# yakovdan/Background-Subtraction

Measured on NVIDIA B200. Metric: frames/s decomposed, higher is better.
Workload: dtype f32 (state) / exact int8-slice Gram on tcgen05 + f64 eigensolve

## Files before the change

background-subtraction_b200/csrc/gram_i8.cu:

```cuda
#include <cooperative_groups.h>
#include <stdio.h>
#include <math.h>
#include <algorithm>
#include <vector>
#include "common.cuh"
#include "kernels.h"
#include "tma.cuh"

namespace cg = cooperative_groups;

namespace bsub {

constexpr int GI_THREADS = 256;
constexpr int GI_KB = 64;
constexpr int GI_STAGES = 3;
constexpr int GI_FLUSH_KB = 448;
constexpr int GI_TILE_BYTES = 128 * GI_KB;
constexpr int GI_STAGE_BYTES = 8 * GI_TILE_BYTES;

struct GramI8Args {
    int n, nblk;
    const int4* cta_info;
    int nkb;
    const int* blk_n;
// ... 204 lines not shown
    asm volatile("{\n\t.reg .pred e;\n\telect.sync _|e, 0xffffffff;\n\t"
                 "@e tcgen05.commit.cta_group::1.mbarrier::arrive::one.shared::cluster.multicast::cluster.b64 [%0], %1;\n\t}"
                 ::"r"(smem_u32(bar)), "h"(cta_mask) : "memory");
}

__global__ void __launch_bounds__(GI_THREADS, 1)
gram_i8_c3_kernel(const __grid_constant__ CUtensorMap mapQ, GramI8C3Args a) {
    if (a.st != nullptr && (a.st->done || a.st->gram_mode != a.require_mode)) return;
    cg::cluster_group cluster = cg::this_cluster();
    extern __shared__ __align__(1024) unsigned char gi_smem[];
    unsigned char* stages = gi_smem;
    uint64_t* full = reinterpret_cast<uint64_t*>(gi_smem + (size_t)GI_STAGES * GI_STAGE_BYTES);
    uint64_t* empty = full + GI_STAGES;
    uint64_t* mine = empty + GI_STAGES;
    uint64_t* tmem_full = mine + GI_STAGES;
    uint64_t* tmem_empty = tmem_full + 1;
    uint32_t* tmem_base_s = reinterpret_cast<uint32_t*>(tmem_empty + 1);

    const int warp = __shfl_sync(0xffffffffu, (int)(threadIdx.x >> 5), 0), lane = threadIdx.x & 31;
    const int rank = (int)cluster.block_rank();
    const int cid = blockIdx.x / 3;
    const bool tX = cid < a.nX;
    const int kb0 = tX ? cid : cid - a.nX, kstride = tX ? a.nX : a.nY;
    const int nkb = (a.nkb > kb0) ? (a.nkb - kb0 + kstride - 1) / kstride : 0;
    const int bi = tX ? (rank == 2 ? 1 : 0) : rank;
    const int bj = tX ? (rank == 0 ? 1 : 2) : rank;
    const bool diag = !tX;
    int ld0_slot, ld0_blk, ld1_slot = -1, ld1_blk = 0; uint16_t ld0_mask, ld1_mask = 0;
    uint16_t sup_mask; int n_consumers;
    if (tX) {
        if (rank == 0)      { ld0_slot = 0; ld0_blk = 0; ld0_mask = 0x3; ld1_slot = 1; ld1_blk = 1; ld1_mask = 0x1; sup_mask = 0x1; n_consumers = 2; }
        else if (rank == 1) { ld0_slot = 1; ld0_blk = 2; ld0_mask = 0x6; sup_mask = 0x3; n_consumers = 2; }
        else                { ld0_slot = 0; ld0_blk = 1; ld0_mask = 0x4; sup_mask = 0x6; n_consumers = 1; }
    } else { ld0_slot = 0; ld0_blk = rank; ld0_mask = (uint16_t)(1u << rank); sup_mask = ld0_mask; n_consumers = 1; }

    if (threadIdx.x == 0) {
        for (int s = 0; s < GI_STAGES; ++s) { mbar_init(&full[s], 1); mbar_init(&empty[s], n_consumers); mbar_init(&mine[s], 1); }
        mbar_init(tmem_full, 1);
        mbar_init(tmem_empty, 128);
        mbar_fence_init();
        tma_prefetch_desc(&mapQ);
    }
    if (warp == 2) {
        asm volatile("tcgen05.alloc.cta_group::1.sync.aligned.shared::cta.b32 [%0], %1;" ::"r"(smem_u32(tmem_base_s)), "r"(512u) : "memory");
        asm volatile("tcgen05.relinquish_alloc_permit.cta_group::1.sync.aligned;" ::: "memory");
    }
    asm volatile("tcgen05.fence::before_thread_sync;" ::: "memory");
    cluster.sync();
    asm volatile("tcgen05.fence::after_thread_sync;" ::: "memory");
    const uint32_t tmem_base = __shfl_sync(0xffffffffu, *tmem_base_s, 0);

    if (warp == 0) {
        if (lane == 0) {
            const uint32_t tx = (uint32_t)(tX ? 8 : 4) * GI_TILE_BYTES;
            for (int kb = 0; kb < nkb; ++kb) {
                const int s = kb % GI_STAGES;
                const int u = kb / GI_STAGES;
                if (u > 0) gi_mbar_wait(&mine[s], (uint32_t)((u - 1) & 1));
                mbar_expect_tx(&full[s], tx);
                if (u > 0) gi_mbar_wait(&empty[s], (uint32_t)((u - 1) & 1));
                unsigned char* base = stages + (size_t)s * GI_STAGE_BYTES;
                const int k16 = (kb0 + kb * kstride) * (GI_KB / 16);
                for (int sl = 0; sl < 4; ++sl)
                    gi_tma_load_3d_mc(base + (size_t)(ld0_slot * 4 + sl) * GI_TILE_BYTES, &mapQ, &full[s], ld0_blk * 2 * a.nb, k16, sl, ld0_mask);
                if (ld1_slot >= 0)
                    for (int sl = 0; sl < 4; ++sl)
                        gi_tma_load_3d_mc(base + (size_t)(ld1_slot * 4 + sl) * GI_TILE_BYTES, &mapQ, &full[s], ld1_blk * 2 * a.nb, k16, sl, ld1_mask);
            }
        }
        __syncwarp();
    } else if (warp == 1) {
        {
            const uint32_t idesc = gi_instr_desc(a.N);
            const uint32_t offB = diag ? 0u : (uint32_t)(4 * GI_TILE_BYTES);
            const uint64_t desc0 = gi_smem_desc(0u, 2048u);
            int since_flush = 0, nflush = 0;
            for (int kb = 0; kb < nkb; ++kb) {
                const int s = kb % GI_STAGES;
                const int u = kb / GI_STAGES;
                if (since_flush == 0 && nflush > 0) {
                    gi_mbar_wait_w(tmem_empty, (uint32_t)((nflush - 1) & 1));
                    asm volatile("tcgen05.fence::after_thread_sync;" ::: "memory");
                }
                gi_mbar_wait_w(&full[s], (uint32_t)(u & 1));
                asm volatile("tcgen05.fence::after_thread_sync;" ::: "memory");
                const uint32_t sbase = smem_u32(stages + (size_t)s * GI_STAGE_BYTES);
                const uint64_t sa = desc0 + (uint64_t)((sbase >> 4) & 0x3FFF), sb = desc0 + (uint64_t)(((sbase + offB) >> 4) & 0x3FFF);
                if (!diag) {
#pragma unroll
                    for (int ks = 0; ks < GI_KB / 32; ++ks) {
#pragma unroll
                        for (int i = 0; i < 4; ++i)
#pragma unroll
                            for (int j = 0; j < 4; ++j) {
                                const int cls = i + j - 3;
                                if (cls < 0) continue;
                                const uint64_t da = sa + (uint64_t)((i * GI_TILE_BYTES + ks * 4096) >> 4);
                                const uint64_t db = sb + (uint64_t)((j * GI_TILE_BYTES + ks * 4096) >> 4);
                                const bool first = (since_flush == 0 && ks == 0 && j == 3);
                                gi_mma_w(tmem_base + (uint32_t)(cls * 128), da, db, idesc, first ? 0u : 1u);
                            }
                    }
                } else {
#pragma unroll
                    for (int ks = 0; ks < GI_KB / 32; ++ks) {
#pragma unroll
                        for (int i = 0; i < 4; ++i)
#pragma unroll
                            for (int j = 0; j < 4; ++j) {
                                const int cls = i + j - 3;
                                if (cls < 0) continue;
                                if (cls != 1 && i > j) continue;
                                const uint64_t da = sa + (uint64_t)((i * GI_TILE_BYTES + ks * 4096) >> 4);
                                const uint64_t db = sb + (uint64_t)((j * GI_TILE_BYTES + ks * 4096) >> 4);
                                const bool first = (since_flush == 0 && ks == 0 && j == 3);
                                gi_mma_w(tmem_base + (uint32_t)(cls * 128), da, db, idesc, first ? 0u : 1u);
                            }
                    }
                }
                gi_commit_mc_w(&empty[s], sup_mask);
                gi_commit_w(&mine[s]);
                ++since_flush;
                if (since_flush == GI_FLUSH_KB || kb == nkb - 1) {
                    gi_commit_w(tmem_full);
                    since_flush = 0; ++nflush;
                }
            }
        }
        __syncwarp();
    } else if (warp >= 4) {
        const int ew = warp - 4;
        const int nflush_total = (nkb + GI_FLUSH_KB - 1) / GI_FLUSH_KB;
        const int lrow = ew * 32 + lane;
        const int row = bi * a.nb + lrow;
        const bool row_ok = lrow < a.nb && row < a.n;
        const size_t ldg = (size_t)3 * 128;
        for (int fl = 0; fl < nflush_total; ++fl) {
            gi_mbar_wait(tmem_full, (uint32_t)(fl & 1));
            asm volatile("tcgen05.fence::after_thread_sync;" ::: "memory");
            for (int c0 = 0; c0 < a.N; c0 += 16) {
                uint32_t v3[16], v4[16], v5[16], v6[16];
                const uint32_t ta = tmem_base + ((uint32_t)(ew * 32) << 16) + (uint32_t)c0;
                gi_tmem_ld16(ta + 0 * 128, v3);
                gi_tmem_ld16(ta + 1 * 128, v4);
                gi_tmem_ld16(ta + 2 * 128, v5);
                gi_tmem_ld16(ta + 3 * 128, v6);
                asm volatile("tcgen05.wait::ld.sync.aligned;" ::: "memory");
                if (row_ok) {
#pragma unroll
                    for (int e = 0; e < 16; ++e) {
                        const int lcol = c0 + e, col = bj * a.nb + lcol;
                        if (lcol < a.nb && col < a.n) {
                            const long long half = (long long)(int)v3[e] + ((long long)(int)v5[e] << 16);
                            const long long whole = ((long long)(int)v4[e] << 8) + ((long long)(int)v6[e] << 24);
                            const long long val = half + whole;
                            if (val != 0) atomicAdd(a.Gint + (size_t)row * ldg + col, (unsigned long long)val);
                            if (diag && half != 0) atomicAdd(a.Gint + (size_t)col * ldg + row, (unsigned long long)half);
                        }
                    }
                }
            }
            asm volatile("tcgen05.fence::before_thread_sync;" ::: "memory");
            gi_mbar_arrive(tmem_empty);
        }
    }
    asm volatile("tcgen05.fence::before_thread_sync;" ::: "memory");
    cluster.sync();
    if (warp == 2) {
        asm volatile("tcgen05.dealloc.cta_group::1.sync.aligned.b32 %0, %1;" ::"r"(tmem_base), "r"(512u) : "memory");
    }
}

__global__ void __launch_bounds__(256) quantize_D_kernel(const float* __restrict__ D, long long ld, int n, long long ldq,
                                                         signed char* __restrict__ Wq, const double* __restrict__ dmax, DevState* st) {
    constexpr int QD_F = 32, QD_KB = 16;
    __shared__ uint4 stage[4][QD_KB][QD_F + 1];
    const double mx = *dmax;
    const double S = (mx > 0.0) ? exp2(ceil(log2(2.0 * mx))) : 1.0;
    if (blockIdx.x == 0 && threadIdx.x == 0) st->wq_scale = S;
    const float Qf = (float)(2147483648.0 / S);
    const long long nkb = ldq / 16, plane = ldq * (long long)n;
    const long long ntk = (nkb + QD_KB - 1) / QD_KB;
    const int ntf = (n + QD_F - 1) / QD_F;
    const long long ntiles = ntk * ntf;
    for (long long tile = blockIdx.x; tile < ntiles; tile += gridDim.x) {
        const long long kb0 = (tile / ntf) * QD_KB;
        const int f0 = (int)(tile % ntf) * QD_F;
#pragma unroll
        for (int pass = 0; pass < 8; ++pass) {
            const int idx = pass * 256 + threadIdx.x;
            const int fl = idx >> 6, q4 = idx & 63;
            const int f = f0 + fl;
            const long long p = kb0 * 16 + 4 * q4;
            float4 d = make_float4(0.f, 0.f, 0.f, 0.f);
            if (f < n && p < ld) d = ldg4_stream(D + (size_t)f * ld + p);
            const unsigned int u0 = ((unsigned int)__float2int_rn(d.x * Qf) + 0x00808080u) ^ 0x00808080u;
            const unsigned int u1 = ((unsigned int)__float2int_rn(d.y * Qf) + 0x00808080u) ^ 0x00808080u;
            const unsigned int u2 = ((unsigned int)__float2int_rn(d.z * Qf) + 0x00808080u) ^ 0x00808080u;
            const unsigned int u3 = ((unsigned int)__float2int_rn(d.w * Qf) + 0x00808080u) ^ 0x00808080u;
// ... 49 lines not shown
GramI8Plan make_gram_i8_plan(int n, long long ldq, int num_sms) {
    GramI8Plan p;
    p.n = n; p.ldq = ldq; p.m_real = 0; p.m_global = 0;
    p.nblk = (n + 127) / 128;
    p.nkb = (int)(ldq / GI_KB);
    p.smem_bytes = (size_t)GI_STAGES * GI_STAGE_BYTES + 256 + 1024;
    p.grid = num_sms;
    return p;
}

void fill_gram_i8_tables(const GramI8Plan& p, std::vector<int4>& cta_info, std::vector<int>& blk_n) {
    blk_n.assign(p.nblk, 128);
    const int last = p.n - (p.nblk - 1) * 128;
    blk_n[p.nblk - 1] = std::min(128, ((last + 15) / 16) * 16);
    std::vector<std::pair<int, int>> tiles;
    std::vector<double> w;
    double wsum = 0.0;
    for (int bi = 0; bi < p.nblk; ++bi)
        for (int bj = bi; bj < p.nblk; ++bj) {
            const double cost = 0.5 * (128.0 + (bi == bj ? 0.0 : (double)blk_n[bj])) / 256.0 +
                                0.5 * (bi == bj ? 0.7 : 1.0) * (double)blk_n[bj] / 128.0;
            tiles.push_back({bi, bj}); w.push_back(cost); wsum += cost;
        }
    std::vector<int> cnt(tiles.size(), 1);
    int left = p.grid - (int)tiles.size();
    if (left < 0) left = 0;
    std::vector<double> want(tiles.size());
    int given = 0;
    for (size_t t = 0; t < tiles.size(); ++t) { want[t] = w[t] / wsum * left; cnt[t] += (int)want[t]; given += (int)want[t]; }
    while (given < left) {
        size_t best = 0; double br = -1.0;
        for (size_t t = 0; t < tiles.size(); ++t) { double r = want[t] - (int)want[t]; if (r > br) { br = r; best = t; } }
        cnt[best]++; want[best] = (int)want[best]; ++given;
    }
    cta_info.clear();
    for (size_t t = 0; t < tiles.size(); ++t) {
        const int c = std::min(cnt[t], std::max(1, p.nkb));
        for (int k = 0; k < c; ++k) cta_info.push_back(make_int4(tiles[t].first, tiles[t].second, k, c));
    }
}

int gram_i8_last_block_n(const GramI8Plan& p) {
    const int last = p.n - (p.nblk - 1) * 128;
    return std::min(128, ((last + 15) / 16) * 16);
}

int make_gram_i8_map(const GramI8Plan& p, const signed char* Wq, CUtensorMap* map, int box_frames) {
    const uint64_t dims[3] = {(uint64_t)2 * p.n, (uint64_t)(p.ldq / 16), 4};
    const uint64_t strides[2] = {(uint64_t)16 * p.n, (uint64_t)p.ldq * (uint64_t)p.n};
    const uint32_t box[3] = {(uint32_t)(2 * box_frames), 4, 1};
    return make_tensor_map_u64(map, Wq, 3, dims, strides, box);
}

static int g_last_block_frames = 128;
int gram_i8_last_block_frames() { return g_last_block_frames; }

int launch_gram_i8(const GramI8Plan& p, const CUtensorMap& map, const CUtensorMap& map_last, const int4* cta_info_dev, int ncta, const int* blk_n_dev,
                   unsigned long long* Gint, double* G, int npad, const DevState* st, double scale_override, int require_mode,
                   cudaStream_t stream) {
    static unsigned long long attr_devs = 0;
    if (first_call_on_device(&attr_devs)) {
        BSUB_CUDA_CHECK(cudaFuncSetAttribute(gram_i8_kernel, cudaFuncAttributeMaxDynamicSharedMemorySize, (int)p.smem_bytes));
    }
    const double E_d = 5461.5 + 128.0 + 65536.0 * 5461.5 + 131072.0 * 0.25, E_o = 6.2e8;
    const double mg = (double)std::max(p.m_global, p.m_real);
    const double err_units = (p.m_real > 0) ? ((double)p.m_real / sqrt(mg)) * ((double)p.n + 3.0 * sqrt((double)p.n)) * E_o * 0x1p-24 : 0.0;
    const double diag_bias = (p.m_real > 0) ? (double)p.m_real * E_d * 0x1p-24 - err_units : 0.0;
    const size_t gbytes = sizeof(unsigned long long) * (size_t)p.nblk * 128 * p.nblk * 128;
    BSUB_CUDA_CHECK(cudaMemsetAsync(Gint, 0, gbytes, stream));
    static int c3_clusters = -1;
    if (p.nblk == 3 && c3_clusters != 0) {
        cudaLaunchConfig_t cfg = {};
        cudaLaunchAttribute at[1];
        at[0].id = cudaLaunchAttributeClusterDimension;
        at[0].val.clusterDim.x = 3; at[0].val.clusterDim.y = 1; at[0].val.clusterDim.z = 1;
        cfg.blockDim = dim3(GI_THREADS); cfg.dynamicSmemBytes = p.smem_bytes; cfg.stream = stream; cfg.attrs = at; cfg.numAttrs = 1;
        if (c3_clusters < 0) {
            c3_clusters = 0;
            if (getenv("BSUB_NO_GRAM_CLUSTER") == nullptr &&
                cudaFuncSetAttribute(gram_i8_c3_kernel, cudaFuncAttributeMaxDynamicSharedMemorySize, (int)p.smem_bytes) == cudaSuccess) {
                cfg.gridDim = dim3(3 * (p.grid / 3));
                int ncl = 0;
                if (cudaOccupancyMaxActiveClusters(&ncl, gram_i8_c3_kernel, &cfg) == cudaSuccess && ncl >= 2) c3_clusters = std::min(ncl, p.grid / 3);
            }
            (void)cudaGetLastError();
            if (getenv("BSUB_DEBUG")) fprintf(stderr, "gram_i8: %d multicast clusters of 3 CTAs\n", c3_clusters);
        }
        if (c3_clusters >= 2) {
            GramI8C3Args c;
            c.n = p.n; c.nkb = p.nkb;
            c.nb = (p.n + 2) / 3; c.N = ((c.nb + 15) / 16) * 16;
            c.nX = std::min(c3_clusters - 1, std::max(1, (int)lround(c3_clusters * 20.0 / 34.0))); c.nY = c3_clusters - c.nX;
            c.Gint = Gint; c.st = st; c.require_mode = require_mode;
            g_last_block_frames = c.nb;
            cfg.gridDim = dim3(3 * c3_clusters);
            BSUB_CUDA_CHECK(cudaLaunchKernelEx(&cfg, gram_i8_c3_kernel, map, c));
            gram_i8_finish_kernel<<<64, 256, 0, stream>>>(Gint, p.nblk, c.nb, p.n, npad, G, st, scale_override, require_mode, diag_bias, err_units,
                                                          (st != nullptr) ? G + (size_t)npad * npad + 8 : nullptr);
            BSUB_CUDA_CHECK(cudaGetLastError());
            return 0;
        }
    }
    GramI8Args a;
    a.n = p.n; a.nblk = p.nblk; a.nkb = p.nkb; a.cta_info = cta_info_dev; a.blk_n = blk_n_dev; a.Gint = Gint; a.st = st; a.require_mode = require_mode;
    gram_i8_kernel<<<ncta, GI_THREADS, p.smem_bytes, stream>>>(map, map_last, a);
    BSUB_CUDA_CHECK(cudaGetLastError());
    g_last_block_frames = 128;
    gram_i8_finish_kernel<<<64, 256, 0, stream>>>(Gint, p.nblk, 128, p.n, npad, G, st, scale_override, require_mode, diag_bias, err_units,
                                                          (st != nullptr) ? G + (size_t)npad * npad + 8 : nullptr);
    BSUB_CUDA_CHECK(cudaGetLastError());
    return 0;
}

}
```

background-subtraction_b200/csrc/kernels.h:

```cpp
#pragma once
#include <cuda.h>
#include <cuda_runtime.h>
#include <stddef.h>
#include <vector>
#include "common.cuh"

namespace bsub {

struct GramPlan {
    int n, npad, nb, ntasks, ntype, gridK, kc, nbox, boxrows;
    long long nchunks;
    size_t smem_bytes, partial_elems;
};
struct GramMaps { CUtensorMap D, S, Y; int narr; };
GramPlan make_gram_plan(int n, long long ld, int num_sms);
void fill_gram_tasks(const GramPlan& p, int2* host_tasks);
int make_gram_maps(const GramPlan& p, const float* D, const float* S, const float* Y, long long ld, GramMaps* maps);
int launch_gram(const GramPlan& p, const GramMaps& maps, bool combo, const int2* dev_tasks, const DevState* st,
                float inv_mu_override, double* partial, double* G, cudaStream_t stream);

struct GramI8Plan { int n, nblk, nkb, grid; long long ldq; size_t smem_bytes;
                    long long m_real;
                    long long m_global; };
GramI8Plan make_gram_i8_plan(int n, long long ldq, int num_sms);
void fill_gram_i8_tables(const GramI8Plan& p, std::vector<int4>& cta_info, std::vector<int>& blk_n);
int make_gram_i8_map(const GramI8Plan& p, const signed char* Wq, CUtensorMap* map, int box_frames);
int gram_i8_last_block_n(const GramI8Plan& p);
int gram_i8_last_block_frames();
int launch_quantize_D(const float* D, long long ld, int n, long long ldq, signed char* Wq, const double* dmax, DevState* st,
                      cudaStream_t stream);
int launch_gram_i8(const GramI8Plan& p, const CUtensorMap& map, const CUtensorMap& map_last, const int4* cta_info_dev, int ncta, const int* blk_n_dev,
                   unsigned long long* Gint, double* G, int npad, const DevState* st, double scale_override, int require_mode,
                   cudaStream_t stream);

struct EigPlan {
    int n, npad, C, rows_per, in_smem, kcap;
    size_t smem_bytes;
    size_t work_doubles;
};
struct EigBuffers {
    double* work;
    double* lam;
    double* Z;
    float* Vr;
    float* VC;
    int vstride;
};
EigPlan make_eig_plan(int n, int npad);
int launch_eig(const EigPlan& p, const double* G, const double* comm_max, EigBuffers b, DevState* st, int mode,
               int k_override, cudaStream_t stream);

struct ShrinkPlan {
    int n, rows, cols, R, P, Cf, nf, threads, grid_clusters, kr;
    long long ld, m;
    int ntile_r, ntile_c;
    long long ntiles;
    size_t smem_bytes;
    size_t tpart_floats;
    int nparts;
};
enum ShrinkMode { SHRINK_FLAT3 = 0, SHRINK_SPILL = 1, SHRINK_L1 = 2 };
ShrinkPlan make_shrink_plan(int n, int rows, int cols, long long ld, int num_sms, int R_hint, int Cf_hint);
struct ShrinkBuffers {
    const float* D; float* S; float* Y;
    float* T;
    float* U;
    float* tpart;
    const float* Vr; const float* VC; int vstride;
    double* part_zz;
    unsigned long long* part_nnz;
    float* part_max;
    float* part_wmax;
    int implied_first = 0;
    int have_flat = 0;
    const float* Tt = nullptr;
};
int launch_shrink(const ShrinkPlan& p, ShrinkBuffers b, const DevState* st, int mode, cudaStream_t stream);

struct ShrinkTmaPlan {
    int n, rows, cols, R, P, Cf, nf, KR, grid_clusters, nparts, ntile_r, ntile_c, bufstride, NT, occ;
    long long ld, ntiles;
    size_t smem_bytes, tpart_floats;
};
struct ShrinkTmaMaps { CUtensorMap D, S, Y, U, Q, Vr, VC; bool has_U, has_Q; };
bool make_shrink_tma_plan(int n, int rows, int cols, long long ld, int num_sms, int R_hint, int Cf_hint, ShrinkTmaPlan* out);
// ... 98 lines not shown
```

background-subtraction_b200/csrc/solver.cu:

```cuda
#include <math.h>
#include <stdarg.h>
#include <stdlib.h>
#include <string.h>
#include <vector>
#include <algorithm>
#include "../../include/bsub_b200.h"
#include "common.cuh"
#include "kernels.h"

namespace bsub {
static thread_local char g_err[1024] = "";
void set_error(const char* fmt, ...) {
    va_list ap;
    va_start(ap, fmt);
    vsnprintf(g_err, sizeof(g_err), fmt, ap);
    va_end(ap);
}
}

using namespace bsub;

#define CK(expr) BSUB_CUDA_CHECK(expr)
#define RET_IF(expr) do { int _rc = (expr); if (_rc != 0) return _rc; } while (0)

static const int kCommTail = 16;
static const int kRunAhead = 3;

struct bsub_solver {
    bsub_config cfg;
    int device = 0, num_sms = 148;
    long long m = 0, ld = 0;
    int n = 0, npad = 0;
    float *D = nullptr, *S = nullptr, *Y = nullptr, *T = nullptr, *L = nullptr, *U = nullptr;
    DevState* st = nullptr;
    IterLog* log = nullptr;
    HostMirror* mirror = nullptr;
    HostMirror* mirror_dev = nullptr;
    double* comm_sum = nullptr;
    double* comm_max = nullptr;
    GramPlan gp; GramMaps gmaps; int2* tasks_dev = nullptr; double* gram_partial = nullptr;
    EigPlan ep; EigBuffers eb;
    ShrinkPlan sp; ShrinkTmaPlan stp; ShrinkTmaMaps stmaps; bool use_tma = false, stmaps_ready = false;
    ShrinkStreamPlan ssp; ShrinkTmaMaps ssmaps; bool use_stream = false;
    bool use_i8 = false; signed char* Wq = nullptr; unsigned long long* Gint = nullptr; GramI8Plan gip; CUtensorMap gimap, gimap_last;
    int4* gi_info = nullptr; int* gi_blkn = nullptr; int gi_ncta = 0; float* part_wmax = nullptr;
    bool use_proj = false; ProjectPlan pjp; float* Tt = nullptr;
    bool use_flat = false, sfmaps_ready = false; ShrinkFlatPlan sfp; ShrinkFlatMaps sfmaps;
    bool force_S = false;
    int proj_iter = -1;
    float* tpart = nullptr; double* part_zz = nullptr; unsigned long long* part_nnz = nullptr;
    float* part_max = nullptr;
    int shrink_mode = SHRINK_FLAT3;
    int* gptr = nullptr; int* gidx = nullptr; int ngroups = 0; bool groups_set = false;
    float* eta_dev = nullptr; float* xi = nullptr; long long xi_floats = 0; float* tot = nullptr;
    float* xi2 = nullptr; float* tot2 = nullptr; int* sweeps2 = nullptr; long long xi2_floats = 0, tot2_floats = 0;
    int* sweeps_dev = nullptr; bool graph_set = false;
    int* pg_ints = nullptr; float* pg_eta = nullptr; GenericGraphDev pg_dev; GenericGraphLayout pg_layout; bool pg_bg = false;
    unsigned char* labels_dev = nullptr; double* lam_table = nullptr; double* bsums = nullptr; int nlab = 0; bool blocks_set = false;
    unsigned char* mask_stage = nullptr;
    double* mask_scratch = nullptr;
    double* stage64 = nullptr; size_t stage64_doubles = 0;
    cudaStream_t last_stream = nullptr; bool stream_seen = false;
    bool implied_first = false;
    bool loaded = false, finalized = false, initialised = false;
    cudaEvent_t ev[kRunAhead + 1];
    int iters_enqueued = 0;
};

static cudaStream_t as_stream(void* s) { return reinterpret_cast<cudaStream_t>(s); }
static cudaStream_t use_stream(bsub_solver* s, void* stream) {
    s->last_stream = as_stream(stream); s->stream_seen = true;
    return s->last_stream;
}
static int ensure_stage64(bsub_solver* s, size_t doubles) {
    if (s->stage64_doubles >= doubles) return 0;
    if (s->stage64) { cudaFree(s->stage64); s->stage64 = nullptr; s->stage64_doubles = 0; }
    BSUB_CUDA_CHECK(cudaMalloc((void**)&s->stage64, sizeof(double) * doubles));
    s->stage64_doubles = doubles;
    return 0;
}
struct DevScope {
    std::vector<void*> ptrs;
    ~DevScope() { for (void* p : ptrs) if (p) cudaFree(p); }
    template <typename T> int alloc(T** out, size_t bytes) {
        void* p = nullptr;
        if (cudaMalloc(&p, bytes ? bytes : 1) != cudaSuccess) { set_error("cudaMalloc(%zu) failed: %s", bytes, cudaGetErrorString(cudaGetLastError())); return -1; }
        ptrs.push_back(p);
        *out = reinterpret_cast<T*>(p);
        return 0;
    }
};

static int round_half_even_005(int d) {
    return (int)nearbyint(0.05 * (double)d);
}

extern "C" {
// ... 82 lines not shown
        if (make_gram_maps(s->gp, s->D, s->S, s->Y, s->ld, &s->gmaps) != 0) { rc = -1; break; }
        std::vector<int2> tasks(s->gp.ntasks);
        fill_gram_tasks(s->gp, tasks.data());
        ALLOC(s->tasks_dev, sizeof(int2) * s->gp.ntasks);
        cudaMemcpy(s->tasks_dev, tasks.data(), sizeof(int2) * s->gp.ntasks, cudaMemcpyHostToDevice);
        ALLOC(s->gram_partial, sizeof(double) * s->gp.partial_elems);
        s->ep = make_eig_plan(s->n, s->npad);
        ALLOC(s->eb.work, sizeof(double) * s->ep.work_doubles);
        ALLOC(s->eb.lam, sizeof(double) * s->n);
        ALLOC(s->eb.Z, sizeof(double) * (size_t)s->n * s->n);
        s->eb.vstride = std::max(16, ((s->n + 3) / 4) * 4);
        ALLOC(s->eb.Vr, sizeof(float) * (size_t)s->n * s->eb.vstride);
        ALLOC(s->eb.VC, sizeof(float) * (size_t)s->n * s->eb.vstride);
        cudaMemset(s->eb.Vr, 0, sizeof(float) * (size_t)s->n * s->eb.vstride);
        cudaMemset(s->eb.VC, 0, sizeof(float) * (size_t)s->n * s->eb.vstride);
        int rows = cfg->rows, cols = cfg->cols;
        if ((long long)rows * cols != s->m) {
            rows = (int)s->m; cols = 1;
            for (int r = 4096; r >= 48; r -= 4)
                if (s->m % r == 0) { rows = r; cols = (int)(s->m / r); break; }
        }
        s->sp = make_shrink_plan(s->n, rows, cols, s->ld, s->num_sms, cfg->tile_rows, cfg->cluster_frames);
        s->use_tma = (getenv("BSUB_NO_TMA") == nullptr) &&
                     make_shrink_tma_plan(s->n, rows, cols, s->ld, s->num_sms, cfg->tile_rows, cfg->cluster_frames, &s->stp);
        s->use_stream = s->use_tma && (getenv("BSUB_NO_STREAM") == nullptr) &&
                        make_shrink_stream_plan(s->n, rows, cols, s->ld, s->num_sms, cfg->tile_rows, &s->ssp);
        ALLOC(s->tpart, sizeof(float) * std::max(s->sp.tpart_floats, s->use_tma ? s->stp.tpart_floats : (size_t)0));
        int nparts = std::max(std::max(s->sp.nparts, (s->use_tma ? s->stp.nparts : 0) + (s->use_stream ? s->ssp.nparts : 0) + s->num_sms), s->num_sms * 8);
        ALLOC(s->part_zz, sizeof(double) * nparts); ALLOC(s->part_nnz, sizeof(unsigned long long) * nparts);
        ALLOC(s->part_max, sizeof(float) * nparts);
        cudaMemset(s->part_zz, 0, sizeof(double) * nparts); cudaMemset(s->part_nnz, 0, sizeof(unsigned long long) * nparts);
        cudaMemset(s->part_max, 0, sizeof(float) * nparts);
        s->use_i8 = s->use_stream && (shrink_stream_ldq(s->ssp) > 0) && (getenv("BSUB_NO_I8") == nullptr) &&
                    (cfg->prox == BSUB_PROX_FLAT_LINF || cfg->prox == BSUB_PROX_L1);
        if (s->use_i8) {
            const long long ldq = shrink_stream_ldq(s->ssp);
            s->gip = make_gram_i8_plan(s->n, ldq, s->num_sms);
            s->gip.m_real = (getenv("BSUB_NO_GRAM_BIAS") == nullptr) ? s->m : 0;
            s->gip.m_global = s->cfg.m_global;
            std::vector<int4> info; std::vector<int> blkn;
            fill_gram_i8_tables(s->gip, info, blkn);
            s->gi_ncta = (int)info.size();
            ALLOC(s->Wq, (size_t)4 * s->n * ldq);
            cudaMemset(s->Wq, 0, (size_t)4 * s->n * ldq);
            ALLOC(s->Gint, sizeof(unsigned long long) * (size_t)s->gip.nblk * 128 * s->gip.nblk * 128);
            ALLOC(s->gi_info, sizeof(int4) * info.size());
            ALLOC(s->gi_blkn, sizeof(int) * blkn.size());
            ALLOC(s->part_wmax, sizeof(float) * (s->ssp.grid + s->num_sms));
            cudaMemcpy(s->gi_info, info.data(), sizeof(int4) * info.size(), cudaMemcpyHostToDevice);
            cudaMemcpy(s->gi_blkn, blkn.data(), sizeof(int) * blkn.size(), cudaMemcpyHostToDevice);
            cudaMemset(s->part_wmax, 0, sizeof(float) * (s->ssp.grid + s->num_sms));
            if (make_gram_i8_map(s->gip, s->Wq, &s->gimap, 128) != 0) { rc = -1; break; }
            if (make_gram_i8_map(s->gip, s->Wq, &s->gimap_last, gram_i8_last_block_n(s->gip)) != 0) { rc = -1; break; }
            s->use_proj = (getenv("BSUB_NO_PROJ") == nullptr) && make_project_plan(s->n, s->ssp.R, ldq, s->num_sms, &s->pjp);
            if (s->use_proj) {
                const size_t tt = sizeof(float) * (size_t)s->ssp.ntiles * 16 * 4 * s->ssp.R;
                ALLOC(s->Tt, tt);
                cudaMemset(s->Tt, 0, tt);
                s->use_flat = (getenv("BSUB_NO_FLAT") == nullptr) && make_shrink_flat_plan(s->n, s->ssp.rows, s->ssp.cols, s->ld, s->num_sms, s->ssp, &s->sfp);
            }
        }
        for (int i = 0; i <= kRunAhead; ++i)
            if (cudaEventCreateWithFlags(&s->ev[i], cudaEventDisableTiming) != cudaSuccess) { set_error("bsub_create: event"); rc = -1; break; }
        if (rc) break;
        switch (cfg->prox) {
            case BSUB_PROX_FLAT_LINF: s->shrink_mode = (cfg->group_rows == 3 && cfg->group_cols == 3) ? SHRINK_FLAT3 : SHRINK_SPILL; break;
            case BSUB_PROX_L1: s->shrink_mode = SHRINK_L1; break;
            default: s->shrink_mode = SHRINK_SPILL; break;
        }
        s->implied_first = s->use_i8 && s->use_stream && s->shrink_mode != SHRINK_SPILL && s->cfg.use_sv_prediction &&
                           s->cfg.sv0 >= 1 && s->cfg.sv0 <= s->ssp.kcap && getenv("BSUB_NO_IMPLIED_FIRST") == nullptr;
        if (s->shrink_mode == SHRINK_SPILL) { ALLOC(s->U, mat); ALLOC(s->L, mat); cudaMemset(s->U, 0, mat); cudaMemset(s->L, 0, mat); }
#undef ALLOC
        if (cudaGetLastError() != cudaSuccess) {  }
    } while (0);
    if (rc != 0) { bsub_destroy(s); return rc; }
    *out = s;
    return 0;
}

int bsub_set_flat_groups(bsub_solver* s, const int32_t* g) {
    if (!s || !g) { set_error("bsub_set_flat_groups: null argument"); return -1; }
    if (s->cfg.prox != BSUB_PROX_FLAT_LINF) { set_error("bsub_set_flat_groups: solver was not created with BSUB_PROX_FLAT_LINF"); return -1; }
    const long long m = s->m;
    const int rows = s->cfg.rows, cols = s->cfg.cols;
    bool regular = ((long long)rows * cols == m);
    if (regular) {
        const int ntr = (rows + 2) / 3;
        for (int j = 0; j < cols && regular; ++j)
            for (int i = 0; i < rows; ++i)
                if (g[(long long)j * rows + i] != (j / 3) * ntr + (i / 3) + 1) { regular = false; break; }
    }
    s->groups_set = true;
    if (regular) { s->shrink_mode = SHRINK_FLAT3; return 0; }
    int gmax = 0;
    for (long long p = 0; p < m; ++p) { if (g[p] < 0) { set_error("bsub_set_flat_groups: negative group id"); return -1; } gmax = std::max(gmax, (int)g[p]); }
    std::vector<int> ptr((size_t)gmax + 1, 0), idx;
    for (long long p = 0; p < m; ++p) if (g[p] > 0) ptr[g[p]]++;
    std::vector<int> start((size_t)gmax + 1, 0);
    int acc = 0;
    for (int k = 1; k <= gmax; ++k) { start[k - 1] = acc; acc += ptr[k]; }
    start[gmax] = acc;
    idx.resize((size_t)std::max(acc, 1));
    std::vector<int> fill(start.begin(), start.end());
    for (long long p = 0; p < m; ++p) if (g[p] > 0) idx[fill[g[p] - 1]++] = (int)p;
    if (s->gptr) cudaFree(s->gptr);
// ... 184 lines not shown
    memset(&h, 0, sizeof(h));
    const bsub_config& c = s->cfg;
    const double mx = (double)std::max<long long>(c.m_global, c.n);
    h.lambda = 1.0 / (sqrt(mx) * c.delta);
    h.non_block_lambda = c.non_block_lambda_scale * h.lambda;
    h.rho = c.rho; h.tol = c.tol; h.mu_scale = c.mu_scale;
    h.max_iter = c.max_iter;
    h.d = c.d_global > 0 ? c.d_global : (int)std::min<long long>(c.m_global, c.n);
    h.round005d = round_half_even_005(h.d);
    h.use_sv_prediction = c.use_sv_prediction;
    h.break_on_rank0 = c.break_on_rank0;
    h.sv = c.use_sv_prediction ? c.sv0 : h.d;
    h.use_i8 = s->use_i8 ? 1 : 0;
    CK(cudaMemcpyAsync(s->st, &h, sizeof(h), cudaMemcpyHostToDevice, st));
    CK(cudaStreamSynchronize(st));
    memset((void*)s->mirror, 0, sizeof(HostMirror));
    return 0;
}

int bsub_set_always_store_S(bsub_solver* s, int on) {
    if (!s) { set_error("bsub_set_always_store_S: null solver"); return -1; }
    s->force_S = on != 0;
    return 0;
}

int bsub_comm_buffers(bsub_solver* s, double** sum_buf, int64_t* sum_count, double** max_buf, int64_t* max_count) {
    if (!s) { set_error("bsub_comm_buffers: null solver"); return -1; }
    if (sum_buf) *sum_buf = s->comm_sum;
    if (sum_count) *sum_count = (int64_t)s->npad * s->npad + kCommTail;
    if (max_buf) *max_buf = s->comm_max;
    if (max_count) *max_count = 8;
    return 0;
}

static int check_ready(bsub_solver* s) {
    if (!s) { set_error("null solver"); return -1; }
    if (!s->loaded) { set_error("no data loaded (call bsub_load_* first)"); return -1; }
    if (s->cfg.prox == BSUB_PROX_FLAT_LINF && !s->groups_set) { set_error("one of graphs or groups must not be None"); return -1; }
    if ((s->cfg.prox == BSUB_PROX_GRAPH_LINF || s->cfg.prox == BSUB_PROX_GRAPH_CENTER_BG || s->cfg.prox == BSUB_PROX_GRAPH_GENERIC) &&
        !s->graph_set) { set_error("one of graphs or groups must not be None"); return -1; }
    if (s->cfg.prox == BSUB_PROX_BLOCK_L2 && !s->blocks_set) { set_error("blocks_by_frame / lambdas_by_frame not set"); return -1; }
    return 0;
}

int bsub_step_init_local(bsub_solver* s, void* stream) {
    RET_IF(check_ready(s));
    cudaStream_t st = use_stream(s, stream);
    RET_IF(upload_state(s, st));
    CK(cudaMemsetAsync(s->comm_max, 0, sizeof(double) * 8, st));
    CK(cudaMemsetAsync(s->comm_sum + (size_t)s->npad * s->npad, 0, sizeof(double) * kCommTail, st));
    RET_IF(launch_rowsum_max(s->D, s->ld, s->m, s->n, s->comm_max, st));
    if (s->use_i8) {
        RET_IF(launch_quantize_D(s->D, s->ld, s->n, s->gip.ldq, s->Wq, s->comm_max + 2, s->st, st));
        RET_IF(launch_gram_i8(s->gip, s->gimap, s->gimap_last, s->gi_info, s->gi_ncta, s->gi_blkn, s->Gint, s->comm_sum, s->npad, s->st, 0.0, 0,
                              st));
    } else {
        RET_IF(launch_gram(s->gp, s->gmaps, false, s->tasks_dev, nullptr, 0.f, s->gram_partial, s->comm_sum, st));
    }
    s->iters_enqueued = 0;
    s->proj_iter = -1;
    s->finalized = false;
    return 0;
}

int bsub_step_init_finish(bsub_solver* s, void* stream) {
    RET_IF(check_ready(s));
    cudaStream_t st = use_stream(s, stream);
    RET_IF(launch_eig(s->ep, s->comm_sum, s->comm_max, s->eb, s->st, 0, 1, st));
    if (!s->implied_first) RET_IF(launch_init_Y(s->D, s->Y, s->S, s->ld, s->n, s->st, st));
    s->initialised = true;
    return 0;
}

int bsub_step_gram(bsub_solver* s, void* stream) {
    if (!s || !s->initialised) { set_error("bsub_step_gram: solver not initialised"); return -1; }
    use_stream(s, stream);
    RET_IF(launch_gram(s->gp, s->gmaps, true, s->tasks_dev, s->st, 0.f, s->gram_partial, s->comm_sum, as_stream(stream)));
    if (s->use_i8)
        RET_IF(launch_gram_i8(s->gip, s->gimap, s->gimap_last, s->gi_info, s->gi_ncta, s->gi_blkn, s->Gint, s->comm_sum, s->npad, s->st, 0.0, 1,
                              as_stream(stream)));
    return 0;
}

int bsub_step_solve(bsub_solver* s, void* stream) {
    if (!s || !s->initialised) { set_error("bsub_step_solve: solver not initialised"); return -1; }
    return launch_eig(s->ep, s->comm_sum, s->comm_max, s->eb, s->st, 1, 0, as_stream(stream));
}

int bsub_step_project(bsub_solver* s, void* stream) {
    if (!s || !s->initialised) { set_error("bsub_step_project: solver not initialised"); return -1; }
    cudaStream_t st = use_stream(s, stream);
    const bool proj = s->use_proj && s->use_stream && s->use_i8 && s->shrink_mode != SHRINK_SPILL;
    if (!proj || s->proj_iter == s->iters_enqueued) return 0;
    RET_IF(launch_project(s->pjp, s->Wq, s->eb.Vr, s->eb.vstride, s->T, s->ld, s->Tt, s->ssp.rows, s->ssp.cols, s->ssp.R, s->ssp.ntile_r,
                          s->ssp.ntiles, s->ssp.kcap, s->st, st));
    s->proj_iter = s->iters_enqueued;
    return 0;
}

static int step_shrink_impl(bsub_solver* s, void* stream, int part) {
    if (!s || !s->initialised) { set_error("bsub_step_shrink: solver not initialised"); return -1; }
    cudaStream_t st = use_stream(s, stream);
    const bool split = s->shrink_mode == SHRINK_SPILL && (s->cfg.prox == BSUB_PROX_BLOCK_L2 || s->cfg.prox == BSUB_PROX_GRAPH_LINF);
    if (part == 2 && !split) return 0;
    if (part == 2) {
        if (s->cfg.prox == BSUB_PROX_BLOCK_L2)
            RET_IF(launch_block_l2_apply(s->U, s->S, s->labels_dev, s->ld, s->m, s->n, s->nlab, s->bsums, s->lam_table, s->st, 0.0, 0.0, st));
        const int np2 = s->num_sms * 8;
        RET_IF(launch_dual_update(s->D, s->S, s->S, s->Y, s->T, s->eb.VC, s->eb.vstride, s->st, s->L, s->ld, s->n, s->part_zz,
                                  s->part_nnz, s->part_max, np2, st));
        RET_IF(launch_control_post(s->st, s->part_zz, s->part_nnz, s->part_max, np2, s->comm_sum + (size_t)s->npad * s->npad, s->log,
                                   s->mirror_dev, 1 | 4, nullptr, 0, st));
        return 0;
    }
    ShrinkBuffers b;
    b.D = s->D; b.S = s->S; b.Y = s->Y; b.T = s->T; b.U = s->U; b.tpart = s->tpart; b.Vr = s->eb.Vr; b.VC = s->eb.VC;
    b.vstride = s->eb.vstride; b.part_zz = s->part_zz; b.part_nnz = s->part_nnz; b.part_max = s->part_max;
    b.part_wmax = s->use_i8 ? s->part_wmax : nullptr;
    b.implied_first = s->implied_first ? 1 : 0;
    const bool proj = s->use_proj && s->use_stream && s->use_i8 && s->shrink_mode != SHRINK_SPILL;
    const bool flat = proj && s->use_flat;
    b.Tt = proj ? s->Tt : nullptr;
    b.have_flat = flat ? 1 : 0;
    int nparts = s->sp.nparts;
    if (s->use_tma) {
        if (!s->stmaps_ready) {
            RET_IF(make_shrink_tma_maps(s->stp, s->D, s->S, s->Y, s->U, &s->stmaps));
            if (s->use_stream) RET_IF(make_shrink_stream_maps(s->ssp, s->D, s->S, s->Y, s->U, &s->ssmaps));
            if (s->use_stream) RET_IF(make_shrink_stream_vmaps(s->ssp, s->eb.Vr, s->eb.VC, s->eb.vstride, &s->ssmaps));
            if (s->use_stream && s->use_i8) RET_IF(make_shrink_stream_qmap(s->ssp, s->Wq, &s->ssmaps));
            s->stmaps_ready = true;
        }
// ... 457 lines not shown

int bsub_gram_dev(const float* D, const float* S, const float* Y, int64_t ld, int64_t m, int32_t n, double mu, double* G_host,
                  void* stream) {
    if (!D || !G_host || ld < m || (ld % 32) != 0) { set_error("bsub_gram_dev: bad argument (ld must be a multiple of 32, pad columns zero)"); return -1; }
    if ((S == nullptr) != (Y == nullptr)) { set_error("bsub_gram_dev: S and Y must both be given or both be NULL"); return -1; }
    cudaStream_t st = as_stream(stream);
    int dev = 0, sms = 148;
    CK(cudaGetDevice(&dev));
    cudaDeviceGetAttribute(&sms, cudaDevAttrMultiProcessorCount, dev);
    GramPlan gp = make_gram_plan(n, ld, sms);
    std::vector<int2> tasks(gp.ntasks);
    fill_gram_tasks(gp, tasks.data());
    DevScope mem;
    int2* tasks_d = nullptr; double *partial = nullptr, *G = nullptr;
    RET_IF(mem.alloc(&tasks_d, sizeof(int2) * gp.ntasks));
    RET_IF(mem.alloc(&partial, sizeof(double) * gp.partial_elems));
    RET_IF(mem.alloc(&G, sizeof(double) * (size_t)gp.npad * gp.npad));
    CK(cudaMemcpy(tasks_d, tasks.data(), sizeof(int2) * gp.ntasks, cudaMemcpyHostToDevice));
    GramMaps gm;
    RET_IF(make_gram_maps(gp, D, S, Y, ld, &gm));
    RET_IF(launch_gram(gp, gm, S != nullptr, tasks_d, nullptr, (float)(S ? 1.0 / mu : 0.0), partial, G, st));
    CK(cudaMemcpy2DAsync(G_host, sizeof(double) * n, G, sizeof(double) * gp.npad, sizeof(double) * n, n, cudaMemcpyDeviceToHost, st));
    CK(cudaStreamSynchronize(st));
    return 0;
}

int bsub_gram_i8_test(const int8_t* slices_host, int32_t n, int64_t ldq, int64_t* G_host) {
    if (!slices_host || !G_host || n <= 0 || ldq <= 0 || (ldq % 64) != 0) { set_error("bsub_gram_i8_test: bad argument"); return -1; }
    int dev = 0, sms = 148;
    CK(cudaGetDevice(&dev));
    cudaDeviceGetAttribute(&sms, cudaDevAttrMultiProcessorCount, dev);
    GramI8Plan gp = make_gram_i8_plan(n, ldq, sms);
    std::vector<int4> info; std::vector<int> blkn;
    fill_gram_i8_tables(gp, info, blkn);
    DevScope mem;
    signed char* q = nullptr; int4* info_d = nullptr; int* blkn_d = nullptr; unsigned long long* Gint = nullptr; double* G = nullptr;
    const size_t qbytes = (size_t)4 * n * ldq, gn = (size_t)gp.nblk * 128;
    const int npad = ((n + 31) / 32) * 32;
    RET_IF(mem.alloc(&q, qbytes));
    RET_IF(mem.alloc(&info_d, sizeof(int4) * info.size()));
    RET_IF(mem.alloc(&blkn_d, sizeof(int) * blkn.size()));
    RET_IF(mem.alloc(&Gint, sizeof(unsigned long long) * gn * gn));
    RET_IF(mem.alloc(&G, sizeof(double) * (size_t)npad * npad));
    {
        std::vector<signed char> packed(qbytes);
        for (int sl = 0; sl < 4; ++sl)
            for (int f = 0; f < n; ++f)
                for (long long k = 0; k < ldq / 16; ++k)
                    memcpy(&packed[(((size_t)sl * (ldq / 16) + k) * n + f) * 16], &slices_host[((size_t)sl * n + f) * ldq + k * 16], 16);
        CK(cudaMemcpy(q, packed.data(), qbytes, cudaMemcpyHostToDevice));
    }
    CK(cudaMemcpy(info_d, info.data(), sizeof(int4) * info.size(), cudaMemcpyHostToDevice));
    CK(cudaMemcpy(blkn_d, blkn.data(), sizeof(int) * blkn.size(), cudaMemcpyHostToDevice));
    CUtensorMap map, map_last;
    RET_IF(make_gram_i8_map(gp, q, &map, 128));
    RET_IF(make_gram_i8_map(gp, q, &map_last, gram_i8_last_block_n(gp)));
    RET_IF(launch_gram_i8(gp, map, map_last, info_d, (int)info.size(), blkn_d, Gint, G, npad, nullptr, 1.0, 1, 0));
    CK(cudaDeviceSynchronize());
    std::vector<long long> tmp(gn * gn);
    CK(cudaMemcpy(tmp.data(), Gint, sizeof(long long) * gn * gn, cudaMemcpyDeviceToHost));
    for (int i = 0; i < n; ++i)
        for (int j = 0; j < n; ++j) {
            const int blk = gram_i8_last_block_frames();
            const int r = (i / blk <= j / blk) ? i : j, c = (i / blk <= j / blk) ? j : i;
            G_host[(size_t)i * n + j] = tmp[(size_t)r * gn + c];
        }
    return 0;
}

int bsub_gram_i8_bench(int32_t n, int64_t ldq, int32_t reps, float* ms_out) {
    if (!ms_out || n <= 0 || ldq <= 0 || (ldq % 64) != 0 || reps <= 0) { set_error("bsub_gram_i8_bench: bad argument"); return -1; }
    int dev = 0, sms = 148;
    CK(cudaGetDevice(&dev));
    cudaDeviceGetAttribute(&sms, cudaDevAttrMultiProcessorCount, dev);
    GramI8Plan gp = make_gram_i8_plan(n, ldq, sms);
    std::vector<int4> info; std::vector<int> blkn;
    fill_gram_i8_tables(gp, info, blkn);
    DevScope mem;
    signed char* q = nullptr; int4* info_d = nullptr; int* blkn_d = nullptr; unsigned long long* Gint = nullptr; double* G = nullptr;
    const size_t qbytes = (size_t)4 * n * ldq, gn = (size_t)gp.nblk * 128;
    const int npad = ((n + 31) / 32) * 32;
    RET_IF(mem.alloc(&q, qbytes));
    RET_IF(mem.alloc(&info_d, sizeof(int4) * info.size()));
    RET_IF(mem.alloc(&blkn_d, sizeof(int) * blkn.size()));
    RET_IF(mem.alloc(&Gint, sizeof(unsigned long long) * gn * gn));
    RET_IF(mem.alloc(&G, sizeof(double) * ((size_t)npad * npad + 16)));
    CK(cudaMemset(q, 0x35, qbytes));
    CK(cudaMemcpy(info_d, info.data(), sizeof(int4) * info.size(), cudaMemcpyHostToDevice));
    CK(cudaMemcpy(blkn_d, blkn.data(), sizeof(int) * blkn.size(), cudaMemcpyHostToDevice));
    CUtensorMap map, map_last;
    RET_IF(make_gram_i8_map(gp, q, &map, 128));
    RET_IF(make_gram_i8_map(gp, q, &map_last, gram_i8_last_block_n(gp)));
    cudaEvent_t e0, e1;
    CK(cudaEventCreate(&e0)); CK(cudaEventCreate(&e1));
    for (int r = 0; r < 2; ++r) RET_IF(launch_gram_i8(gp, map, map_last, info_d, (int)info.size(), blkn_d, Gint, G, npad, nullptr, 1.0, 1, 0));
    CK(cudaEventRecord(e0, 0));
    for (int r = 0; r < reps; ++r) RET_IF(launch_gram_i8(gp, map, map_last, info_d, (int)info.size(), blkn_d, Gint, G, npad, nullptr, 1.0, 1, 0));
    CK(cudaEventRecord(e1, 0));
    CK(cudaEventSynchronize(e1));
    float ms = 0.f;
    CK(cudaEventElapsedTime(&ms, e0, e1));
    cudaEventDestroy(e0); cudaEventDestroy(e1);
    *ms_out = ms / (float)reps;
    return 0;
}

int bsub_eig_topk(const double* G_host, int32_t n, int32_t k, double* lam_host, double* vec_host) {
    if (!G_host || n <= 0 || k <= 0 || k > n || !lam_host) { set_error("bsub_eig_topk: bad argument"); return -1; }
    const int npad = ((n + 31) / 32) * 32;
    EigPlan ep = make_eig_plan(n, npad);
    EigBuffers eb;
    memset(&eb, 0, sizeof(eb));
    DevScope mem;
    double* G = nullptr; DevState* st = nullptr;
    RET_IF(mem.alloc(&G, sizeof(double) * (size_t)npad * npad));
    CK(cudaMemset(G, 0, sizeof(double) * (size_t)npad * npad));
    CK(cudaMemcpy2D(G, sizeof(double) * npad, G_host, sizeof(double) * n, sizeof(double) * n, n, cudaMemcpyHostToDevice));
    RET_IF(mem.alloc(&eb.work, sizeof(double) * ep.work_doubles));
    RET_IF(mem.alloc(&eb.lam, sizeof(double) * n));
    RET_IF(mem.alloc(&eb.Z, sizeof(double) * (size_t)n * n));
    RET_IF(mem.alloc(&st, sizeof(DevState)));
    CK(cudaMemset(st, 0, sizeof(DevState)));
    eb.vstride = n;
    RET_IF(launch_eig(ep, G, nullptr, eb, st, 2, k, 0));
    CK(cudaDeviceSynchronize());
    CK(cudaMemcpy(lam_host, eb.lam, sizeof(double) * k, cudaMemcpyDeviceToHost));
    if (vec_host) CK(cudaMemcpy(vec_host, eb.Z, sizeof(double) * (size_t)k * n, cudaMemcpyDeviceToHost));
    return 0;
}

}
```

Before: 3279.

## Merge int8-slice Gram MMAs into wider N tiles with single TMA per block

```diff
diff --git a/background-subtraction_b200/csrc/gram_i8.cu b/background-subtraction_b200/csrc/gram_i8.cu
--- a/background-subtraction_b200/csrc/gram_i8.cu
+++ b/background-subtraction_b200/csrc/gram_i8.cu
@@ -280,7 +280,7 @@
 
     if (warp == 0) {
         if (lane == 0) {
-            const uint32_t tx = (uint32_t)(tX ? 8 : 4) * GI_TILE_BYTES;
+            const uint32_t tx = (uint32_t)(tX ? 2 : 1) * 256u * (uint32_t)a.N;
             for (int kb = 0; kb < nkb; ++kb) {
                 const int s = kb % GI_STAGES;
                 const int u = kb / GI_STAGES;
@@ -289,19 +289,18 @@
                 if (u > 0) gi_mbar_wait(&empty[s], (uint32_t)((u - 1) & 1));
                 unsigned char* base = stages + (size_t)s * GI_STAGE_BYTES;
                 const int k16 = (kb0 + kb * kstride) * (GI_KB / 16);
-                for (int sl = 0; sl < 4; ++sl)
-                    gi_tma_load_3d_mc(base + (size_t)(ld0_slot * 4 + sl) * GI_TILE_BYTES, &mapQ, &full[s], ld0_blk * 2 * a.nb, k16, sl, ld0_mask);
+                gi_tma_load_3d_mc(base + (size_t)ld0_slot * 4 * GI_TILE_BYTES, &mapQ, &full[s], ld0_blk * 2 * a.nb, 0, k16, ld0_mask);
                 if (ld1_slot >= 0)
-                    for (int sl = 0; sl < 4; ++sl)
-                        gi_tma_load_3d_mc(base + (size_t)(ld1_slot * 4 + sl) * GI_TILE_BYTES, &mapQ, &full[s], ld1_blk * 2 * a.nb, k16, sl, ld1_mask);
+                    gi_tma_load_3d_mc(base + (size_t)ld1_slot * 4 * GI_TILE_BYTES, &mapQ, &full[s], ld1_blk * 2 * a.nb, 0, k16, ld1_mask);
             }
         }
         __syncwarp();
     } else if (warp == 1) {
         {
-            const uint32_t idesc = gi_instr_desc(a.N);
+            const uint32_t idesc1 = gi_instr_desc(a.N), idesc2 = gi_instr_desc(2 * a.N);
             const uint32_t offB = diag ? 0u : (uint32_t)(4 * GI_TILE_BYTES);
-            const uint64_t desc0 = gi_smem_desc(0u, 2048u);
+            const uint64_t desc0 = gi_smem_desc(0u, 64u * (uint32_t)a.N);
+            const uint32_t cN = (uint32_t)a.N;
             int since_flush = 0, nflush = 0;
             for (int kb = 0; kb < nkb; ++kb) {
                 const int s = kb % GI_STAGES;
@@ -314,36 +313,20 @@
                 asm volatile("tcgen05.fence::after_thread_sync;" ::: "memory");
                 const uint32_t sbase = smem_u32(stages + (size_t)s * GI_STAGE_BYTES);
                 const uint64_t sa = desc0 + (uint64_t)((sbase >> 4) & 0x3FFF), sb = desc0 + (uint64_t)(((sbase + offB) >> 4) & 0x3FFF);
-                if (!diag) {
-#pragma unroll
-                    for (int ks = 0; ks < GI_KB / 32; ++ks) {
-#pragma unroll
-                        for (int i = 0; i < 4; ++i)
-#pragma unroll
-                            for (int j = 0; j < 4; ++j) {
-                                const int cls = i + j - 3;
-                                if (cls < 0) continue;
-                                const uint64_t da = sa + (uint64_t)((i * GI_TILE_BYTES + ks * 4096) >> 4);
-                                const uint64_t db = sb + (uint64_t)((j * GI_TILE_BYTES + ks * 4096) >> 4);
-                                const bool first = (since_flush == 0 && ks == 0 && j == 3);
-                                gi_mma_w(tmem_base + (uint32_t)(cls * 128), da, db, idesc, first ? 0u : 1u);
-                            }
-                    }
-                } else {
-#pragma unroll
-                    for (int ks = 0; ks < GI_KB / 32; ++ks) {
-#pragma unroll
-                        for (int i = 0; i < 4; ++i)
-#pragma unroll
-                            for (int j = 0; j < 4; ++j) {
-                                const int cls = i + j - 3;
-                                if (cls < 0) continue;
-                                if (cls != 1 && i > j) continue;
-                                const uint64_t da = sa + (uint64_t)((i * GI_TILE_BYTES + ks * 4096) >> 4);
-                                const uint64_t db = sb + (uint64_t)((j * GI_TILE_BYTES + ks * 4096) >> 4);
-                                const bool first = (since_flush == 0 && ks == 0 && j == 3);
-                                gi_mma_w(tmem_base + (uint32_t)(cls * 128), da, db, idesc, first ? 0u : 1u);
-                            }
+#pragma unroll
+                for (int ks = 0; ks < GI_KB / 32; ++ks) {
+                    const uint64_t ka = sa + (uint64_t)(8 * ks) * cN, kbd = sb + (uint64_t)(8 * ks) * cN;
+                    const uint32_t acc0 = (since_flush == 0 && ks == 0) ? 0u : 1u;
+                    gi_mma_w(tmem_base + 0 * cN, ka + 3 * cN, kbd + 0 * cN, idesc2, acc0);
+                    gi_mma_w(tmem_base + 2 * cN, ka + 3 * cN, kbd + 2 * cN, idesc2, acc0);
+                    if (!diag) {
+                        gi_mma_w(tmem_base + 0 * cN, ka + 2 * cN, kbd + 1 * cN, idesc2, 1u);
+                        gi_mma_w(tmem_base + 2 * cN, ka + 2 * cN, kbd + 3 * cN, idesc1, 1u);
+                        gi_mma_w(tmem_base + 0 * cN, ka + 1 * cN, kbd + 2 * cN, idesc2, 1u);
+                        gi_mma_w(tmem_base + 0 * cN, ka + 0 * cN, kbd + 3 * cN, idesc1, 1u);
+                    } else {
+                        gi_mma_w(tmem_base + 0 * cN, ka + 2 * cN, kbd + 1 * cN, idesc2, 1u);
+                        gi_mma_w(tmem_base + 1 * cN, ka + 1 * cN, kbd + 3 * cN, idesc1, 1u);
                     }
                 }
                 gi_commit_mc_w(&empty[s], sup_mask);
@@ -369,10 +352,11 @@
             for (int c0 = 0; c0 < a.N; c0 += 16) {
                 uint32_t v3[16], v4[16], v5[16], v6[16];
                 const uint32_t ta = tmem_base + ((uint32_t)(ew * 32) << 16) + (uint32_t)c0;
-                gi_tmem_ld16(ta + 0 * 128, v3);
-                gi_tmem_ld16(ta + 1 * 128, v4);
-                gi_tmem_ld16(ta + 2 * 128, v5);
-                gi_tmem_ld16(ta + 3 * 128, v6);
+                const uint32_t cN = (uint32_t)a.N;
+                gi_tmem_ld16(ta + 0 * cN, v3);
+                gi_tmem_ld16(ta + 1 * cN, v4);
+                gi_tmem_ld16(ta + 2 * cN, v5);
+                gi_tmem_ld16(ta + 3 * cN, v6);
                 asm volatile("tcgen05.wait::ld.sync.aligned;" ::: "memory");
                 if (row_ok) {
 #pragma unroll
@@ -528,10 +512,22 @@
     return make_tensor_map_u64(map, Wq, 3, dims, strides, box);
 }
 
+int gram_i8_c3_N(int n) { return ((((n + 2) / 3) + 15) / 16) * 16; }
+
+int make_gram_i8_c3_map(const GramI8Plan& p, const signed char* Wq, CUtensorMap* map) {
+    if (p.nblk != 3) { *map = CUtensorMap{}; return 0; }
+    const int N = gram_i8_c3_N(p.n);
+    const uint64_t dims[3] = {(uint64_t)2 * p.n, 4, (uint64_t)(p.ldq / 16)};
+    const uint64_t strides[2] = {(uint64_t)p.ldq * (uint64_t)p.n, (uint64_t)16 * p.n};
+    const uint32_t box[3] = {(uint32_t)(2 * N), 4, 4};
+    return make_tensor_map_u64(map, Wq, 3, dims, strides, box);
+}
+
 static int g_last_block_frames = 128;
 int gram_i8_last_block_frames() { return g_last_block_frames; }
 
-int launch_gram_i8(const GramI8Plan& p, const CUtensorMap& map, const CUtensorMap& map_last, const int4* cta_info_dev, int ncta, const int* blk_n_dev,
+int launch_gram_i8(const GramI8Plan& p, const CUtensorMap& map, const CUtensorMap& map_last, const CUtensorMap& map_c3, const int4* cta_info_dev,
+                   int ncta, const int* blk_n_dev,
                    unsigned long long* Gint, double* G, int npad, const DevState* st, double scale_override, int require_mode,
                    cudaStream_t stream) {
     static unsigned long long attr_devs = 0;
@@ -565,12 +561,12 @@
         if (c3_clusters >= 2) {
             GramI8C3Args c;
             c.n = p.n; c.nkb = p.nkb;
-            c.nb = (p.n + 2) / 3; c.N = ((c.nb + 15) / 16) * 16;
+            c.nb = (p.n + 2) / 3; c.N = gram_i8_c3_N(p.n);
             c.nX = std::min(c3_clusters - 1, std::max(1, (int)lround(c3_clusters * 20.0 / 34.0))); c.nY = c3_clusters - c.nX;
             c.Gint = Gint; c.st = st; c.require_mode = require_mode;
             g_last_block_frames = c.nb;
             cfg.gridDim = dim3(3 * c3_clusters);
-            BSUB_CUDA_CHECK(cudaLaunchKernelEx(&cfg, gram_i8_c3_kernel, map, c));
+            BSUB_CUDA_CHECK(cudaLaunchKernelEx(&cfg, gram_i8_c3_kernel, map_c3, c));
             gram_i8_finish_kernel<<<64, 256, 0, stream>>>(Gint, p.nblk, c.nb, p.n, npad, G, st, scale_override, require_mode, diag_bias, err_units,
                                                           (st != nullptr) ? G + (size_t)npad * npad + 8 : nullptr);
             BSUB_CUDA_CHECK(cudaGetLastError());
diff --git a/background-subtraction_b200/csrc/kernels.h b/background-subtraction_b200/csrc/kernels.h
--- a/background-subtraction_b200/csrc/kernels.h
+++ b/background-subtraction_b200/csrc/kernels.h
@@ -25,12 +25,14 @@
 GramI8Plan make_gram_i8_plan(int n, long long ldq, int num_sms);
 void fill_gram_i8_tables(const GramI8Plan& p, std::vector<int4>& cta_info, std::vector<int>& blk_n);
 int make_gram_i8_map(const GramI8Plan& p, const signed char* Wq, CUtensorMap* map, int box_frames);
+int make_gram_i8_c3_map(const GramI8Plan& p, const signed char* Wq, CUtensorMap* map);
+int gram_i8_c3_N(int n);
 int gram_i8_last_block_n(const GramI8Plan& p);
 int gram_i8_last_block_frames();
 int launch_quantize_D(const float* D, long long ld, int n, long long ldq, signed char* Wq, const double* dmax, DevState* st,
                       cudaStream_t stream);
-int launch_gram_i8(const GramI8Plan& p, const CUtensorMap& map, const CUtensorMap& map_last, const int4* cta_info_dev, int ncta, const int* blk_n_dev,
-                   unsigned long long* Gint, double* G, int npad, const DevState* st, double scale_override, int require_mode,
+int launch_gram_i8(const GramI8Plan& p, const CUtensorMap& map, const CUtensorMap& map_last, const CUtensorMap& map_c3, const int4* cta_info_dev,
+                   int ncta, const int* blk_n_dev, unsigned long long* Gint, double* G, int npad, const DevState* st, double scale_override, int require_mode,
                    cudaStream_t stream);
 
 struct EigPlan {
diff --git a/background-subtraction_b200/csrc/solver.cu b/background-subtraction_b200/csrc/solver.cu
--- a/background-subtraction_b200/csrc/solver.cu
+++ b/background-subtraction_b200/csrc/solver.cu
@@ -42,7 +42,7 @@
     EigPlan ep; EigBuffers eb;
     ShrinkPlan sp; ShrinkTmaPlan stp; ShrinkTmaMaps stmaps; bool use_tma = false, stmaps_ready = false;
     ShrinkStreamPlan ssp; ShrinkTmaMaps ssmaps; bool use_stream = false;
-    bool use_i8 = false; signed char* Wq = nullptr; unsigned long long* Gint = nullptr; GramI8Plan gip; CUtensorMap gimap, gimap_last;
+    bool use_i8 = false; signed char* Wq = nullptr; unsigned long long* Gint = nullptr; GramI8Plan gip; CUtensorMap gimap, gimap_last, gimap_c3;
     int4* gi_info = nullptr; int* gi_blkn = nullptr; int gi_ncta = 0; float* part_wmax = nullptr;
     bool use_proj = false; ProjectPlan pjp; float* Tt = nullptr;
     bool use_flat = false, sfmaps_ready = false; ShrinkFlatPlan sfp; ShrinkFlatMaps sfmaps;
@@ -231,6 +231,7 @@
             cudaMemset(s->part_wmax, 0, sizeof(float) * (s->ssp.grid + s->num_sms));
             if (make_gram_i8_map(s->gip, s->Wq, &s->gimap, 128) != 0) { rc = -1; break; }
             if (make_gram_i8_map(s->gip, s->Wq, &s->gimap_last, gram_i8_last_block_n(s->gip)) != 0) { rc = -1; break; }
+            if (make_gram_i8_c3_map(s->gip, s->Wq, &s->gimap_c3) != 0) { rc = -1; break; }
             s->use_proj = (getenv("BSUB_NO_PROJ") == nullptr) && make_project_plan(s->n, s->ssp.R, ldq, s->num_sms, &s->pjp);
             if (s->use_proj) {
                 const size_t tt = sizeof(float) * (size_t)s->ssp.ntiles * 16 * 4 * s->ssp.R;
@@ -521,7 +522,7 @@
     RET_IF(launch_rowsum_max(s->D, s->ld, s->m, s->n, s->comm_max, st));
     if (s->use_i8) {
         RET_IF(launch_quantize_D(s->D, s->ld, s->n, s->gip.ldq, s->Wq, s->comm_max + 2, s->st, st));
-        RET_IF(launch_gram_i8(s->gip, s->gimap, s->gimap_last, s->gi_info, s->gi_ncta, s->gi_blkn, s->Gint, s->comm_sum, s->npad, s->st, 0.0, 0,
+        RET_IF(launch_gram_i8(s->gip, s->gimap, s->gimap_last, s->gimap_c3, s->gi_info, s->gi_ncta, s->gi_blkn, s->Gint, s->comm_sum, s->npad, s->st, 0.0, 0,
                               st));
     } else {
         RET_IF(launch_gram(s->gp, s->gmaps, false, s->tasks_dev, nullptr, 0.f, s->gram_partial, s->comm_sum, st));
@@ -546,7 +547,7 @@
     use_stream(s, stream);
     RET_IF(launch_gram(s->gp, s->gmaps, true, s->tasks_dev, s->st, 0.f, s->gram_partial, s->comm_sum, as_stream(stream)));
     if (s->use_i8)
-        RET_IF(launch_gram_i8(s->gip, s->gimap, s->gimap_last, s->gi_info, s->gi_ncta, s->gi_blkn, s->Gint, s->comm_sum, s->npad, s->st, 0.0, 1,
+        RET_IF(launch_gram_i8(s->gip, s->gimap, s->gimap_last, s->gimap_c3, s->gi_info, s->gi_ncta, s->gi_blkn, s->Gint, s->comm_sum, s->npad, s->st, 0.0, 1,
                               as_stream(stream)));
     return 0;
 }
@@ -1110,10 +1111,11 @@
     }
     CK(cudaMemcpy(info_d, info.data(), sizeof(int4) * info.size(), cudaMemcpyHostToDevice));
     CK(cudaMemcpy(blkn_d, blkn.data(), sizeof(int) * blkn.size(), cudaMemcpyHostToDevice));
-    CUtensorMap map, map_last;
+    CUtensorMap map, map_last, map_c3;
     RET_IF(make_gram_i8_map(gp, q, &map, 128));
     RET_IF(make_gram_i8_map(gp, q, &map_last, gram_i8_last_block_n(gp)));
-    RET_IF(launch_gram_i8(gp, map, map_last, info_d, (int)info.size(), blkn_d, Gint, G, npad, nullptr, 1.0, 1, 0));
+    RET_IF(make_gram_i8_c3_map(gp, q, &map_c3));
+    RET_IF(launch_gram_i8(gp, map, map_last, map_c3, info_d, (int)info.size(), blkn_d, Gint, G, npad, nullptr, 1.0, 1, 0));
     CK(cudaDeviceSynchronize());
     std::vector<long long> tmp(gn * gn);
     CK(cudaMemcpy(tmp.data(), Gint, sizeof(long long) * gn * gn, cudaMemcpyDeviceToHost));
@@ -1146,14 +1148,15 @@
     CK(cudaMemset(q, 0x35, qbytes));
     CK(cudaMemcpy(info_d, info.data(), sizeof(int4) * info.size(), cudaMemcpyHostToDevice));
     CK(cudaMemcpy(blkn_d, blkn.data(), sizeof(int) * blkn.size(), cudaMemcpyHostToDevice));
-    CUtensorMap map, map_last;
+    CUtensorMap map, map_last, map_c3;
     RET_IF(make_gram_i8_map(gp, q, &map, 128));
     RET_IF(make_gram_i8_map(gp, q, &map_last, gram_i8_last_block_n(gp)));
+    RET_IF(make_gram_i8_c3_map(gp, q, &map_c3));
     cudaEvent_t e0, e1;
     CK(cudaEventCreate(&e0)); CK(cudaEventCreate(&e1));
-    for (int r = 0; r < 2; ++r) RET_IF(launch_gram_i8(gp, map, map_last, info_d, (int)info.size(), blkn_d, Gint, G, npad, nullptr, 1.0, 1, 0));
+    for (int r = 0; r < 2; ++r) RET_IF(launch_gram_i8(gp, map, map_last, map_c3, info_d, (int)info.size(), blkn_d, Gint, G, npad, nullptr, 1.0, 1, 0));
     CK(cudaEventRecord(e0, 0));
-    for (int r = 0; r < reps; ++r) RET_IF(launch_gram_i8(gp, map, map_last, info_d, (int)info.size(), blkn_d, Gint, G, npad, nullptr, 1.0, 1, 0));
+    for (int r = 0; r < reps; ++r) RET_IF(launch_gram_i8(gp, map, map_last, map_c3, info_d, (int)info.size(), blkn_d, Gint, G, npad, nullptr, 1.0, 1, 0));
     CK(cudaEventRecord(e1, 0));
     CK(cudaEventSynchronize(e1));
     float ms = 0.f;
```

New measurement: 3372, median of 6. 2.9% higher.
